# bennyguo/instant-nsr-pl

Hardware: NVIDIA H100
Metric: rays/sec fwd+bwd (NeRF-Synthetic lego shape) (higher is better)
Workload: dtype f16

## Files before the change

include/nsr_b200.h:

```cpp
#ifndef NSR_B200_H
#define NSR_B200_H
#include <stdint.h>

#ifdef __cplusplus
extern "C" {
#endif

#define NSR_MAX_LEVELS 32
#define NSR_VERSION 100

typedef struct {
  int32_t n_levels;
  int32_t n_features;
  float scale[NSR_MAX_LEVELS];
  uint32_t res[NSR_MAX_LEVELS];
  uint32_t size[NSR_MAX_LEVELS];
  uint32_t offset[NSR_MAX_LEVELS];
  uint32_t dense_mask;
} nsr_grid_t;

typedef struct {
  int32_t n_in;
  int32_t n_out;
  int32_t n_hidden;
// ... 131 lines not shown
                             const int64_t* k_dev, const float* xyzdir, void* denc_h, void* stream);
int nsr_nerf_field_bwd_net(const nsr_nerf_t* f, const void* enc_k_h, const void* dparams_h, const void* cparams_h, const float* d_sraw,
                           const float* d_rgb, float* grad_dparams, float* grad_cparams, float loss_scale, const float* amax, int64_t k,
                           const int64_t* k_dev, const float* xyzdir, void* denc_h, void* stream);
int nsr_nerf_table_scatter(const nsr_grid_t* g, const float* xyz, int32_t stride, const void* denc_h, float loss_scale, const float* amax,
                           float* grad_table, int64_t k, const int64_t* k_dev, int32_t level_begin, int32_t level_end, int32_t ctas_per_sm,
                           void* stream);


int nsr_nerf_rays_fwd(const nsr_nerf_t* f, const float* rays, const uint32_t* masks, int32_t words, const float* t_min,
                      const int64_t* offsets_m, const int32_t* order, float step, float early_stop_eps, const void* dparams_h,
                      const void* cparams_h,
                      void* enc_save_h, float* sigmas, float* rgbs, float* weights, float* trans, int32_t* kidx, float* acc_rgb,
                      float* opacity, float* depth, int32_t* kept, uint32_t* ticket, int64_t n_rays, const int32_t* counts,
                      const int32_t* bin_counts, int32_t* kept_blocks, void* stream);
int nsr_nerf_render_rays(const nsr_nerf_t* f, const nsr_march_t* m, const float* rays, const uint32_t* masks, int32_t words,
                         const float* t_start, const int32_t* counts, const int32_t* bin_counts, const int32_t* order_bins,
                         float early_stop_eps, const void* dparams_h, const void* cparams_h, float* acc_rgb, float* opacity,
                         float* depth, int32_t* kept, uint32_t* ticket, int64_t n_rays, void* stream);
int nsr_pack_kept(const int64_t* offsets_m, const int64_t* offsets_k, const float* t_min, float step, const int32_t* kidx,
                  const float* weights, int32_t* ray_indices_k, float* t_starts_k, float* t_ends_k, float* weights_k ,
                  int64_t* loose_pos ,
                  const nsr_nerf_t* f, const float* rays, const void* enc_loose_h ,
                  void* enc_k_h ,
                  float* xyzdir_k ,
                  int32_t enc_tiled ,
                  int64_t n_rays, void* stream);
int nsr_pack_kept_scan(const int64_t* offsets_m, const int32_t* kept, int64_t* offsets_k_out, const float* t_min, float step,
                       const int32_t* kidx, const float* weights, int32_t* ray_indices_k, float* t_starts_k, float* t_ends_k,
                       float* weights_k, int64_t* loose_pos, const nsr_nerf_t* f, const float* rays, const void* enc_loose_h, void* enc_k_h,
                       float* xyzdir_k, int32_t enc_tiled, int64_t n_rays, const int32_t* kept_blocks, void* stream);
int nsr_nerf_ray_bwd_loose(const int64_t* offsets_m, const int32_t* kept, const float* t_min, float step, const int32_t* kidx, const float* trans,
                           const float* weights, const float* sigmas, const float* rgbs, const float* g_rgb, const float* g_opacity,
                           const float* g_depth, const float* g_weights, float* d_sraw, float* d_rgb, float* amax,
                           const int64_t* offsets_k, int64_t n_rays, void* stream);
int nsr_nerf_rays_bwd(const nsr_nerf_t* f, const float* rays, const float* t_min, const int64_t* offsets_m, const int32_t* kept, float step,
                      const void* enc_save_h, const float* sigmas, const float* rgbs, const float* weights, const float* trans,
                      const int32_t* kidx, const void* dparams_h, const void* cparams_h, const float* g_rgb, const float* g_opacity,
                      const float* g_depth, const float* g_weights, float* grad_dparams, float* grad_cparams, float loss_scale, float* amax,
                      float t_bound, uint32_t* ticket, int64_t n_rays, void* stream);
int nsr_neus_field_fwd(const nsr_grid_t* g, const float* points, const void* table_h, const float* W1, const float* b1, const float* W2,
                       const float* b2, float radius, int32_t n_out, float* sdf, float* grad, float* feature, int64_t n, const int64_t* n_dev,
                       void* stream);
int nsr_neus_field_bwd(const nsr_grid_t* g, const float* points, const void* table_h, const float* W1, const float* b1, const float* W2,
                       const float* b2, float radius, int32_t n_out, const float* g_out, const float* g_sdf, const float* g_grad,
                       const float* amax, float* grad_table, float* dW1, float* db1, float* dW2, float* db2, int64_t n, const int64_t* n_dev,
                       void* stream);
int nsr_neus_field_fwd_levels(const nsr_grid_t* g, const float* points, const void* table_h, const float* W1, const float* b1, const float* W2,
                              const float* b2, float radius, int32_t n_out, const float* n_active, float* sdf, float* grad, float* feature, int64_t n,
                              const int64_t* n_dev, void* stream);
// ... 119 lines not shown
```

instant-nsr-pl_b200/csrc/nerf_rays_fwd.cu:

```cuda
#include "march.cuh"
#include "nerf_fused.cuh"

namespace {

constexpr int kWarps = 8;
constexpr int kThreads = kWarps * 32;
constexpr int kMaxWords = 64;
constexpr int kMaxWordsCone = 96;
constexpr int kWarpHalves = 32 * NF_LD32 + 32 * 24 + 64 + 256;
constexpr size_t kSmemBytes = (size_t)(NF_W_TOTAL + kWarps * kWarpHalves) * sizeof(__half);

struct RaysFwdArgs {
  const float* rays;
  const uint32_t* masks;
  const float* t_min;
  const int64_t* offsets_m;
  const int32_t* order;
  const int32_t* bin_counts;
  const int32_t* counts;
  const __half* dparams;
  const __half* cparams;
  __half* enc_save;
  float* sigmas;
  float* rgbs;
  float* weights;
  float* trans;
  int32_t* kidx_out;
  float* acc_rgb;
  float* opacity;
  float* depth;
  int32_t* kept;
  int32_t* kept_blocks;
  uint32_t* ticket;
  float step, early_stop_eps;
  int words;
  int64_t n_rays;
  float cone;
};

__device__ __forceinline__ float warp_incl_prod(float v, int lane) {
#pragma unroll
  for (int o = 1; o < 32; o <<= 1) {
    const float t = __shfl_up_sync(0xffffffffu, v, o);
    if (lane >= o) v *= t;
  }
  return v;
}
// ... 1 lines not shown
#pragma unroll
  for (int o = 16; o > 0; o >>= 1) v += __shfl_xor_sync(0xffffffffu, v, o);
  return v;
}

constexpr int kMinBlocks = 2;
constexpr int kGatherBatch = 4;
template <bool CONE, bool STORE>
__global__ void __launch_bounds__(kThreads, kMinBlocks) nerf_rays_fwd_kernel(const __grid_constant__ nsr_nerf_t P, const RaysFwdArgs a) {
  extern __shared__ __align__(16) __half smem[];
  const int warp = threadIdx.x >> 5, lane = threadIdx.x & 31, g = lane >> 2, c = lane & 3;
  __half* At = smem + NF_W_TOTAL + warp * kWarpHalves;
  __half* St = At + 32 * NF_LD32;
  float* s_sig = reinterpret_cast<float*>(St + 32 * 24);
  float* s_rgb = s_sig + 32;
  const __half2* table = reinterpret_cast<const __half2*>(a.dparams + NF_DENSITY_PARAMS);
  nf_stage_weights(smem, a.dparams, a.cparams, true);
  __shared__ int bins[NSR_ORDER_BINS];
  if (threadIdx.x < NSR_ORDER_BINS) bins[threadIdx.x] = a.bin_counts != nullptr ? __ldg(a.bin_counts + threadIdx.x) : 0;
  __syncthreads();

  for (;;) {
    int64_t ray = 0;
    if (lane == 0) ray = atomicAdd(a.ticket, 1u);
    ray = __shfl_sync(0xffffffffu, ray, 0);
    if (ray >= a.n_rays) break;
    if (a.bin_counts != nullptr) {
      int t = (int)ray, b = 0;
#pragma unroll
      for (int q = 0; q < NSR_ORDER_BINS - 1; ++q) {
// ... 63 lines not shown
          filled += take;
        }
        const bool valid = k >= 0;
        if (!valid) k = 0;
        const float t0 = CONE ? ct0 : __fmaf_rn((float)k, a.step, tmin), t1 = CONE ? ct1 : __fmaf_rn((float)k + 1.f, a.step, tmin);
        const float mid = (t0 + t1) * 0.5f;
        uint32_t f[16];
        if (valid && CONE) {
          float x = fmaf(dx, mid, ox), y = fmaf(dy, mid, oy), z = fmaf(dz, mid, oz);
          nf_contract<NF_UNBOUNDED_SPHERE>(P, x, y, z);
          nf_gather_batched<16, kGatherBatch>(P.grid, table, x, y, z, f);
        } else if (valid) {
          const float x = (fmaf(dx, mid, ox) + P.radius) * inv, y = (fmaf(dy, mid, oy) + P.radius) * inv,
                      z = (fmaf(dz, mid, oz) + P.radius) * inv;
          nf_gather_batched<16, kGatherBatch>(P.grid, table, x, y, z, f);
        } else {
#pragma unroll
          for (int l = 0; l < 16; ++l) f[l] = 0u;
        }
        nf_store_row32(At, lane, f);
        if (STORE && a.enc_save != nullptr && valid) {
          uint4* e = reinterpret_cast<uint4*>(a.enc_save + (base + s_idx) * 32);
          e[0] = make_uint4(f[0], f[1], f[2], f[3]);
          e[1] = make_uint4(f[4], f[5], f[6], f[7]);
          e[2] = make_uint4(f[8], f[9], f[10], f[11]);
          e[3] = make_uint4(f[12], f[13], f[14], f[15]);
        }
        __syncwarp();
        uint32_t a_o[2][1][4];
        {
// ... 67 lines not shown
          d_acc += w * mid;
          r_acc += w * cr;
          g_acc += w * cg;
          b_acc += w * cb;
          if (STORE) {
            const int64_t p = base + s_idx;
            a.sigmas[p] = sigma;
            a.weights[p] = w;
            a.trans[p] = T;
            a.kidx_out[p] = k;
            a.rgbs[p * 3 + 0] = cr;
            a.rgbs[p * 3 + 1] = cg;
            a.rgbs[p * 3 + 2] = cb;
          }
        }
        kept += __popc(__ballot_sync(0xffffffffu, keep));
        carry *= __shfl_sync(0xffffffffu, incl, 31);
        __syncwarp();
        if (carry < a.early_stop_eps) break;
      }
    }
    o_acc = warp_sum(o_acc);
    d_acc = warp_sum(d_acc);
    r_acc = warp_sum(r_acc);
    g_acc = warp_sum(g_acc);
    b_acc = warp_sum(b_acc);
    if (lane == 0) {
      a.opacity[ray] = o_acc;
      a.depth[ray] = d_acc;
      a.acc_rgb[ray * 3 + 0] = r_acc;
      a.acc_rgb[ray * 3 + 1] = g_acc;
// ... 72 lines not shown
    for (int64_t v = lane; v < cnt * 4; v += 32) {
      const int64_t R = dst + (v >> 2);
      const int kc = (int)(v & 3), r = (int)(R & 127);
      enc_k[(R >> 7) * 512 + ((r >> 3) * 4 + kc) * 8 + (r & 7)] = enc_loose[src * 4 + v];
    }
  }
}

__global__ void __launch_bounds__(256) ray_bwd_loose_kernel(const int64_t* __restrict__ off_m, const int32_t* __restrict__ kept,
                                                            const float* __restrict__ t_min, float step, const int32_t* __restrict__ kidx,
                                                            const float* __restrict__ trans, const float* __restrict__ weights,
                                                            const float* __restrict__ sigmas, const float* __restrict__ rgbs,
                                                            const float* __restrict__ g_rgb, const float* __restrict__ g_opacity,
                                                            const float* __restrict__ g_depth, const float* __restrict__ g_weights,
                                                            float* __restrict__ d_sraw, float* __restrict__ d_rgb, float* __restrict__ amax,
                                                            const int64_t* __restrict__ off_k, int64_t n_rays) {
  const int lane = threadIdx.x & 31;
  const int64_t ray = blockIdx.x * 8ll + (threadIdx.x >> 5);
  if (ray >= n_rays) return;
  const int64_t beg = off_m[ray];
  const int64_t out0 = off_k ? off_k[ray] : beg;
  const int n = kept[ray];
  if (n <= 0) return;
  const float tmin = t_min[ray];
  const float gr = g_rgb ? g_rgb[ray * 3 + 0] : 0.f, gg = g_rgb ? g_rgb[ray * 3 + 1] : 0.f, gb = g_rgb ? g_rgb[ray * 3 + 2] : 0.f;
  const float go = g_opacity ? g_opacity[ray] : 0.f, gd = g_depth ? g_depth[ray] : 0.f;
  float carry = 0.f, vmax = 0.f;
  for (int cb = ((n - 1) / 32) * 32; cb >= 0; cb -= 32) {
    const int j = cb + lane;
    const bool ok = j < n;
    const int64_t i = beg + j;
    float w = 0.f, gi = 0.f, delta = 0.f;
    if (ok) {
      w = weights[i];
      const float kf = (float)kidx[i];
      const float t0 = __fmaf_rn(kf, step, tmin), t1 = __fmaf_rn(kf + 1.f, step, tmin);
      delta = t1 - t0;
      gi = gr * rgbs[i * 3 + 0] + gg * rgbs[i * 3 + 1] + gb * rgbs[i * 3 + 2] + go + gd * ((t0 + t1) * 0.5f) + (g_weights ? g_weights[i] : 0.f);
      d_rgb[(out0 + j) * 3 + 0] = w * gr;
      d_rgb[(out0 + j) * 3 + 1] = w * gg;
      d_rgb[(out0 + j) * 3 + 2] = w * gb;
      vmax = fmaxf(vmax, 0.25f * w * fmaxf(fabsf(gr), fmaxf(fabsf(gg), fabsf(gb))));
    }
    const float gw = gi * w;
    float suf = gw;
#pragma unroll
    for (int o = 1; o < 32; o <<= 1) {
      const float t = __shfl_down_sync(0xffffffffu, suf, o);
      if (lane + o < 32) suf += t;
    }
    if (ok) {
      const float ds = delta * (gi * (trans[i] - w) - (carry + suf - gw));
      const float dr = ds * fminf(sigmas[i], 3269017.37f);
      d_sraw[out0 + j] = dr;
      vmax = fmaxf(vmax, fabsf(dr));
    }
    carry += __shfl_sync(0xffffffffu, suf, 0);
  }
  if (amax != nullptr) {
#pragma unroll
    for (int o = 16; o > 0; o >>= 1) vmax = fmaxf(vmax, __shfl_xor_sync(0xffffffffu, vmax, o));
    if (lane == 0 && vmax > 0.f && isfinite(vmax)) atomicMax(reinterpret_cast<int*>(amax), __float_as_int(vmax));
  }
}

template <bool CONE, bool STORE>
int reserve_smem(const char* name) {
  static thread_local bool attr_set = false;
  if (!attr_set) {
    cudaError_t e = cudaFuncSetAttribute(nerf_rays_fwd_kernel<CONE, STORE>, cudaFuncAttributeMaxDynamicSharedMemorySize, (int)kSmemBytes);
    if (e != cudaSuccess) {
      nsr_set_error("%s: cannot reserve %zu B shared memory: %s", name, kSmemBytes, cudaGetErrorString(e));
      return 2;
    }
    attr_set = true;
  }
  return 0;
}

int rays_grid(int64_t n_rays) {
  const int64_t want = (n_rays + kWarps - 1) / kWarps;
  return (int)min((int64_t)nsr_sm_count() * 2, want > 0 ? want : (int64_t)1);
}

}

extern "C" int nsr_nerf_rays_fwd(const nsr_nerf_t* f, const float* rays, const uint32_t* masks, int32_t words, const float* t_min,
                                 const int64_t* offsets_m, const int32_t* order, float step, float early_stop_eps, const void* dparams_h, const void* cparams_h,
                                 void* enc_save_h, float* sigmas, float* rgbs, float* weights, float* trans, int32_t* kidx,
                                 float* acc_rgb, float* opacity, float* depth, int32_t* kept, uint32_t* ticket, int64_t n_rays,
                                 const int32_t* counts, const int32_t* bin_counts, int32_t* kept_blocks, void* stream) {
  NSR_REQUIRE(bin_counts == nullptr || (order != nullptr && counts != nullptr), "nsr_nerf_rays_fwd: the binned queue needs order [8][n] and counts");
  NSR_REQUIRE(f != nullptr && f->grid.n_levels == 16 && f->grid.n_features == 2 && f->feature_dim == 16 && f->density_hidden == 1 &&
                  f->color_hidden == 2 && f->contraction == 0,
              "nsr_nerf_rays_fwd: fused path needs L=16, F=2, feature_dim=16, hidden layers 1/2, AABB contraction");
  NSR_REQUIRE(words >= 1 && words <= kMaxWords, "nsr_nerf_rays_fwd: words must be in [1,%d]", kMaxWords);
  NSR_REQUIRE(ticket != nullptr && kept != nullptr, "nsr_nerf_rays_fwd: ticket / kept are required");
  if (n_rays == 0) return 0;
  if (int e = reserve_smem<false, true>("nsr_nerf_rays_fwd")) return e;
  RaysFwdArgs a;
  a.rays = rays; a.masks = masks; a.t_min = t_min; a.offsets_m = offsets_m; a.order = order; a.bin_counts = bin_counts; a.counts = counts; a.kept_blocks = kept_blocks;
  a.dparams = (const __half*)dparams_h; a.cparams = (const __half*)cparams_h; a.enc_save = (__half*)enc_save_h;
  a.sigmas = sigmas; a.rgbs = rgbs; a.weights = weights; a.trans = trans; a.kidx_out = kidx;
  a.acc_rgb = acc_rgb; a.opacity = opacity; a.depth = depth; a.kept = kept; a.ticket = ticket;
  a.step = step; a.early_stop_eps = early_stop_eps; a.words = words; a.n_rays = n_rays; a.cone = 0.f;
  nerf_rays_fwd_kernel<false, true><<<rays_grid(n_rays), kThreads, kSmemBytes, (cudaStream_t)stream>>>(*f, a);
  NSR_CHECK_LAUNCH("nsr_nerf_rays_fwd");
  return 0;
}

extern "C" int nsr_nerf_render_rays(const nsr_nerf_t* f, const nsr_march_t* m, const float* rays, const uint32_t* masks, int32_t words,
                                    const float* t_start, const int32_t* counts, const int32_t* bin_counts, const int32_t* order_bins,
                                    float early_stop_eps, const void* dparams_h, const void* cparams_h, float* acc_rgb, float* opacity,
                                    float* depth, int32_t* kept, uint32_t* ticket, int64_t n_rays, void* stream) {
  NSR_REQUIRE(f != nullptr && m != nullptr, "nsr_nerf_render_rays: field / march descriptor is NULL");
  NSR_REQUIRE(f->grid.n_levels == 16 && f->grid.n_features == 2 && f->feature_dim == 16 && f->density_hidden == 1 && f->color_hidden == 2,
              "nsr_nerf_render_rays: needs L=16, F=2, feature_dim=16, hidden layers 1/2");
  NSR_REQUIRE(f->contraction == m->contraction, "nsr_nerf_render_rays: field contraction %d != march contraction %d", f->contraction,
              m->contraction);
  NSR_REQUIRE(f->contraction == NF_AABB || f->contraction == NF_UNBOUNDED_SPHERE,
              "nsr_nerf_render_rays: contraction type %d not implemented (AABB=0, UN_BOUNDED_SPHERE=2)", f->contraction);
  const bool cone = f->contraction == NF_UNBOUNDED_SPHERE;
  NSR_REQUIRE(m->step > 0.f && (cone ? m->cone_angle >= 0.f : m->cone_angle == 0.f),
// ... 56 lines not shown
  dummy.radius = 1.f;
  pack_kept_kernel<true><<<nsr_blocks(n_rays, 8), 256, 0, (cudaStream_t)stream>>>(offsets_m, nullptr, kept, offsets_k_out, t_min, step, kidx, weights,
                                                                                  ray_indices_k, t_starts_k, t_ends_k, weights_k, loose_pos,
                                                                                  f ? *f : dummy, rays, (const uint4*)enc_loose_h,
                                                                                  (uint4*)enc_k_h, xyzdir_k, enc_tiled, n_rays, kept_blocks);
  NSR_CHECK_LAUNCH("nsr_pack_kept_scan");
  return 0;
}

extern "C" int nsr_nerf_ray_bwd_loose(const int64_t* offsets_m, const int32_t* kept, const float* t_min, float step, const int32_t* kidx,
                                      const float* trans, const float* weights, const float* sigmas, const float* rgbs, const float* g_rgb,
                                      const float* g_opacity, const float* g_depth, const float* g_weights, float* d_sraw, float* d_rgb,
                                      float* amax, const int64_t* offsets_k, int64_t n_rays, void* stream) {
  if (n_rays == 0) return 0;
  ray_bwd_loose_kernel<<<nsr_blocks(n_rays, 8), 256, 0, (cudaStream_t)stream>>>(offsets_m, kept, t_min, step, kidx, trans, weights, sigmas, rgbs,
                                                                                g_rgb, g_opacity, g_depth, g_weights, d_sraw, d_rgb, amax, offsets_k, n_rays);
  NSR_CHECK_LAUNCH("nsr_nerf_ray_bwd_loose");
  return 0;
}
```

instant-nsr-pl_b200/fused.py:

```python
import ctypes
import math

import torch

from . import ops
from .lib import lib, ptr, stream, check_cuda, contig, NerfT
from .nerfacc import ContractionType, ray_aabb_intersect

SCATTER_LEVEL_GROUPS = ((12, 16), (8, 12), (0, 8))


class _NerfRender(torch.autograd.Function):

    @staticmethod
    def forward(ctx, fused, rays, jitter, static, *params):
        kp = fused.kernel_params(*params)
        st = fused.trace(rays, jitter, static, kp)
        n_rays, cap = rays.shape[0], st['cap']
        dev = rays.device
        acc_rgb = torch.zeros(n_rays, 3, device=dev)
        opacity = torch.zeros(n_rays, 1, device=dev)
        depth = torch.zeros(n_rays, 1, device=dev)
        sig = torch.empty(cap, device=dev)
        rgbs = torch.empty(cap, 3, device=dev)
# ... 37 lines not shown
        n = rays.shape[0]
        cap = n * fused.cap_per_ray
        mref = ctypes.byref(fused.march)
        u = None
        if m.randomized:
            u = torch.rand(n, device=dev) if jitter is None else contig(jitter.to(dev), torch.float32)
        grid = m.occupancy_grid
        bits, coarse = grid.bits(), grid.coarse_bits()
        i32 = lambda k: torch.empty(k, dtype=torch.int32, device=dev)
        f32 = lambda *k: torch.empty(*k, dtype=torch.float32, device=dev)
        i64 = lambda k: torch.empty(k, dtype=torch.int64, device=dev)
        words = (fused.cap_per_ray + 31) // 32
        need_grad = (dparams.requires_grad or cparams.requires_grad) and fused._want_grad
        masks, t_min, counts = i32(n * words), f32(n), i32(n)
        nb = (n + 255) // 256
        zz = torch.zeros(12 + nb, dtype=torch.int32, device=dev)
        tick, amax0, m_total, bin_counts = zz[0:1], zz[1:2].view(torch.float32), zz[2:4].view(torch.int64), zz[4:12]
        kept_blocks = zz[12:] if fused.fuse_kept_scan else None
        if fused.march_alloc:
            offsets_m, order = i64(n), i32(8 * n)
            lib.call('nsr_march_rays_alloc', mref, ptr(rays), ptr(u), ptr(bits), ptr(coarse), ptr(masks), words, ptr(t_min), ptr(counts), ptr(offsets_m),
                     ptr(m_total), ptr(bin_counts), ptr(order), n, stream())
        else:
            offsets_m, order = i64(n + 1), i32(n)
            lib.call('nsr_march_rays_mask', mref, ptr(rays), ptr(u), ptr(bits), ptr(coarse), ptr(masks), words, ptr(t_min), ptr(counts), n, stream())
            lib.call('nsr_scan_counts_order', ptr(counts), ptr(offsets_m), ptr(order), n, stream())
            m_total = offsets_m[n:]
        enc = torch.empty(cap, 32, dtype=torch.float16, device=dev) if need_grad else None
        sig, rgbs, weights, trans, kidx = f32(cap), f32(cap, 3), f32(cap), f32(cap), i32(cap)
        acc_rgb, opacity, depth, kept = f32(n, 3), f32(n, 1), f32(n, 1), i32(n)
        offsets_k = i64(n + 1)
        dh, ch = fused.dparams_half(), fused.cparams_half()
        step = float(m.render_step_size)
        lib.call('nsr_nerf_rays_fwd', fused.ref(), ptr(rays), ptr(masks), words, ptr(t_min), ptr(offsets_m), ptr(order), step,
                 float(fused.early_stop_eps), ptr(dh), ptr(ch), ptr(enc), ptr(sig), ptr(rgbs), ptr(weights), ptr(trans), ptr(kidx),
                 ptr(acc_rgb), ptr(opacity), ptr(depth), ptr(kept), ptr(tick), n, ptr(counts), ptr(bin_counts) if fused.march_alloc else None, ptr(kept_blocks), stream())
        if not fused.fuse_kept_scan:
            lib.call('nsr_scan_counts', ptr(kept), ptr(offsets_k), n, stream())
        ri, ts, te, pos = i32(cap), f32(cap), f32(cap), i64(cap)
        packed_bwd = need_grad and fused.bwd_kernel in ('tiles', 'tiles_split', 'tc') and fused.packed_bwd_inputs
        tiled = 1 if fused.bwd_kernel == 'tc' else 0
        pad = 256 - cap % 128 if tiled else 64
        enc_k = torch.empty(cap + pad, 32, dtype=torch.float16, device=dev) if packed_bwd else None
        xyzdir = f32(cap + pad, 6) if packed_bwd else None
        if fused.fuse_kept_scan:
            lib.call('nsr_pack_kept_scan', ptr(offsets_m), ptr(kept), ptr(offsets_k), ptr(t_min), step, ptr(kidx), ptr(weights), ptr(ri), ptr(ts),
                     ptr(te), None, ptr(pos), fused.ref(), ptr(rays), ptr(enc), ptr(enc_k), ptr(xyzdir), tiled, n, ptr(kept_blocks), stream())
        else:
            lib.call('nsr_pack_kept', ptr(offsets_m), ptr(offsets_k), ptr(t_min), step, ptr(kidx), ptr(weights), ptr(ri), ptr(ts), ptr(te), None,
                     ptr(pos), fused.ref(), ptr(rays), ptr(enc), ptr(enc_k), ptr(xyzdir), tiled, n, stream())
        ctx.fused, ctx.n_rays, ctx.cap = fused, n, cap
        ctx.set_materialize_grads(False)
        if packed_bwd:
            enc = None
        ctx.save_for_backward(rays, t_min, offsets_m, offsets_k, kept, enc, sig, rgbs, weights, trans, kidx, ri, ts, te, pos, dh, ch,
                              enc_k, xyzdir, amax0)
        ctx.mark_non_differentiable(ri, ts, te, pos, offsets_m, offsets_k, m_total, counts)
        return acc_rgb, opacity, depth, weights, ri, ts, te, pos, offsets_m, offsets_k, m_total, counts

    @staticmethod
    def backward(ctx, g_rgb, g_op, g_depth, g_w, *_):
        fused = ctx.fused
        rays, t_min, offsets_m, offsets_k, kept, enc, sig, rgbs, weights, trans, kidx, ri, ts, te, pos, dh, ch, enc_k, xyzdir, amax0 = ctx.saved_tensors
        dev = rays.device
        n, cap = ctx.n_rays, ctx.cap
        step = float(fused.model.render_step_size)
        direct = fused.direct_grads
        if direct is not None:
            gd, gc = direct
        else:
            gd = torch.empty(fused.n_dparams, device=dev)
            gc = torch.empty(fused.n_cparams, device=dev)
        n_head = fused.net.mlp.n_params
        split = fused.bwd_kernel == 'tiles_split' and enc_k is not None and n > 0
        (gd[:n_head] if split else gd).zero_()
        gc.zero_()
        if (enc is not None or enc_k is not None) and n > 0:
            f32 = lambda t: None if t is None else contig(t, torch.float32)
            amax = amax0
            if fused.bwd_kernel == 'rays':
                tick = torch.zeros(1, dtype=torch.int32, device=dev)
                lib.call('nsr_nerf_rays_bwd', fused.ref(), ptr(rays), ptr(t_min), ptr(offsets_m), ptr(kept), step, ptr(enc), ptr(sig), ptr(rgbs),
                         ptr(weights), ptr(trans), ptr(kidx), ptr(dh), ptr(ch), ptr(f32(g_rgb)), ptr(f32(g_op)), ptr(f32(g_depth)),
                         ptr(f32(g_w)), ptr(gd), ptr(gc), float(fused.loss_scale), ptr(amax), float(fused.t_bound), ptr(tick), n, stream())
            else:
                packed = enc_k is not None
                pad = 256 - cap % 128 if fused.bwd_kernel == 'tc' else 64
                d_sraw = torch.empty(cap + pad, device=dev)
                d_rgb = torch.empty(cap + pad, 3, device=dev)
                lib.call('nsr_nerf_ray_bwd_loose', ptr(offsets_m), ptr(kept), ptr(t_min), step, ptr(kidx), ptr(trans), ptr(weights), ptr(sig),
                         ptr(rgbs), ptr(f32(g_rgb)), ptr(f32(g_op)), ptr(f32(g_depth)), ptr(f32(g_w)), ptr(d_sraw), ptr(d_rgb), ptr(amax),
                         ptr(offsets_k) if packed else None, n, stream())
                if packed and fused.bwd_kernel == 'tc':
                    if fused._tc_status is None or fused._tc_status.device != dev:
                        fused._tc_status = torch.zeros(1, dtype=torch.int32, device=dev)
                    lib.call('nsr_nerf_field_bwd_tc', fused.ref(), ptr(enc_k), ptr(dh), ptr(ch), ptr(d_sraw), ptr(d_rgb), ptr(gd), ptr(gc),
                             float(fused.loss_scale), ptr(amax), cap, ptr(offsets_k[n:]), ptr(xyzdir), ptr(fused._tc_status), stream())
                elif packed and fused.bwd_kernel == 'tiles_split':
                    denc = torch.empty(cap, 32, dtype=torch.float16, device=dev)
                    lib.call('nsr_nerf_field_bwd_net', fused.ref(), ptr(enc_k), ptr(dh), ptr(ch), ptr(d_sraw), ptr(d_rgb), ptr(gd), ptr(gc),
                             float(fused.loss_scale), ptr(amax), cap, ptr(offsets_k[n:]), ptr(xyzdir), ptr(denc), stream())
                    groups = fused.level_groups or SCATTER_LEVEL_GROUPS
                    off = fused.grid.offset
                    if sorted(l for g in groups for l in range(*g)) != list(range(len(off) - 1)):
                        raise ValueError(f'level_groups {groups} must partition the {len(off) - 1} levels: the backward zeroes the table per group')
                    for gi, (l0, l1) in enumerate(groups):
                        gd[n_head + 2 * int(off[l0]):n_head + 2 * int(off[l1])].zero_()
                        lib.call('nsr_nerf_table_scatter', ctypes.byref(fused.struct.grid), ptr(xyzdir), 6, ptr(denc), float(fused.loss_scale), ptr(amax),
                                 ptr(gd[n_head:]), cap, ptr(offsets_k[n:]), l0, l1, 4 if (fused.exchange_hook is not None and gi > 0) else 0,
                                 stream())
                        if fused.exchange_hook is not None:
                            fused.exchange_hook(gi)
                else:
                    lib.call('nsr_nerf_field_bwd', fused.ref(), ptr(rays), ptr(ri), ptr(ts), ptr(te), ptr(enc_k if packed else enc), ptr(dh), ptr(ch),
                             ptr(d_sraw), ptr(d_rgb), ptr(gd), ptr(gc), float(fused.loss_scale), ptr(amax), cap, ptr(offsets_k[n:]),
                             None if packed else ptr(pos), ptr(xyzdir), stream())
        if direct is not None:
            return None, None, None, None, None
        return gd, gc, None, None, None


def nerf_field_struct(grid, radius, density_bias, contraction_type):
    s = NerfT()
    s.grid = grid.struct
# ... 349 lines not shown
```

instant-nsr-pl_b200/lib.py:

```python
import ctypes as C
import os

import torch

HERE = os.path.dirname(os.path.abspath(__file__))
NSR_MAX_LEVELS = 32


class NsrError(RuntimeError):
    pass


def library_path():
    return os.path.join(HERE, 'libnsr_b200.so')


class GridT(C.Structure):
    _fields_ = [('n_levels', C.c_int32), ('n_features', C.c_int32),
                ('scale', C.c_float * NSR_MAX_LEVELS), ('res', C.c_uint32 * NSR_MAX_LEVELS),
                ('size', C.c_uint32 * NSR_MAX_LEVELS), ('offset', C.c_uint32 * NSR_MAX_LEVELS),
                ('dense_mask', C.c_uint32)]


class MlpT(C.Structure):
# ... 44 lines not shown
    'nsr_scan_counts': [P, P, I64, P],
    'nsr_march_write': [P, P, P, P, P, P, P, P, P, P, I64, P],
    'nsr_visibility': [P, P, P, P, P, F32, F32, I64, P],
    'nsr_weight_from_density_fwd': [P, P, P, P, P, P, I64, P],
    'nsr_weight_from_density_bwd': [P, P, P, P, P, P, P, I64, P],
    'nsr_weight_from_alpha_fwd': [P, P, P, P, I64, P],
    'nsr_weight_from_alpha_bwd': [P, P, P, P, P, P, I64, P],
    'nsr_accumulate': [P, P, P, P, I32, I64, P],
    'nsr_march_rays_mask': [P, P, P, P, P, P, I32, P, P, I64, P],
    'nsr_scan_counts_order': [P, P, P, I64, P],
    'nsr_march_rays_alloc': [P, P, P, P, P, P, I32, P, P, P, P, P, P, I64, P],
    'nsr_march_rays_expand': [P, P, I32, P, P, P, P, P, I64, P],
    'nsr_march_cone_mask': [P, P, P, P, P, F32, F32, P, P, I32, P, P, I64, P],
    'nsr_march_cone_expand': [P, P, I32, P, P, P, P, P, I64, P, I64, P],
    'nsr_nerf_rays_fwd': [P, P, P, I32, P, P, P, F32, F32, P, P, P, P, P, P, P, P, P, P, P, P, P, I64, P, P, P, P],
    'nsr_nerf_render_rays': [P, P, P, P, I32, P, P, P, P, F32, P, P, P, P, P, P, P, I64, P],
    'nsr_pack_kept': [P, P, P, F32, P, P, P, P, P, P, P, P, P, P, P, P, I32, I64, P],
    'nsr_pack_kept_scan': [P, P, P, P, F32, P, P, P, P, P, P, P, P, P, P, P, P, I32, I64, P, P],
    'nsr_nerf_ray_bwd_loose': [P, P, P, F32, P, P, P, P, P, P, P, P, P, P, P, P, P, I64, P],
    'nsr_nerf_rays_bwd': [P, P, P, P, P, F32, P, P, P, P, P, P, P, P, P, P, P, P, P, P, F32, P, F32, P, I64, P],
    'nsr_neus_field_fwd': [P, P, P, P, P, P, P, F32, I32, P, P, P, I64, P, P],
    'nsr_neus_field_bwd': [P, P, P, P, P, P, P, F32, I32, P, P, P, P, P, P, P, P, P, I64, P, P],
    'nsr_neus_field_fwd_levels': [P, P, P, P, P, P, P, F32, I32, P, P, P, P, I64, P, P],
    'nsr_neus_field_bwd_levels': [P, P, P, P, P, P, P, F32, I32, P, P, P, P, P, P, P, P, P, P, I64, P, P],
    'nsr_neus_field_fd_fwd': [P, P, P, P, P, P, P, F32, I32, P, P, P, P, P, I64, P, P],
    'nsr_neus_field_fd_bwd': [P, P, P, P, P, P, P, F32, I32, P, P, P, P, P, P, P, P, P, P, I64, P, P],
    'nsr_neus_sdf_lattice': [P, P, P, P, I32, I32, I32, I32, I32, P, P, P, P, P, F32, I32, P, P, P],
    'nsr_absmax3': [P, I64, P, I64, P, I64, P, I64, P, P],
    'nsr_sample_points': [P, P, P, P, P, P, P, I64, P, P],
    'nsr_neus_alpha_fwd': [P, P, P, P, P, F32, P, P, P, I64, P, P],
    'nsr_neus_alpha_bwd': [P, P, P, P, P, F32, P, P, P, P, P, P, I64, P, P],
    'nsr_neus_composite_fwd': [P, P, P, P, P, P, P, P, P, P, P, P, I64, P],
    'nsr_neus_composite_bwd': [P, P, P, P, P, P, P, P, P, P, P, P, P, P, P, P, I64, P],
    'nsr_neus_render_rays': [P, P, P, I32, P, P, P, P, F32, P, P, P, P, P, F32, I32, P, P, I32, P, P, P, P, P, P, P, P, P, I64, P],
# ... 134 lines not shown
```

Baseline: 15.21 million.

## Write packed backward inputs directly from forward kernel via atomic row allocation

```diff
diff --git a/include/nsr_b200.h b/include/nsr_b200.h
--- a/include/nsr_b200.h
+++ b/include/nsr_b200.h
@@ -169,6 +169,12 @@
                       void* enc_save_h, float* sigmas, float* rgbs, float* weights, float* trans, int32_t* kidx, float* acc_rgb,
                       float* opacity, float* depth, int32_t* kept, uint32_t* ticket, int64_t n_rays, const int32_t* counts,
                       const int32_t* bin_counts, int32_t* kept_blocks, void* stream);
+int nsr_nerf_rays_fwd_rows(const nsr_nerf_t* f, const float* rays, const uint32_t* masks, int32_t words, const float* t_min,
+                           const int64_t* offsets_m, const int32_t* order, float step, float early_stop_eps, const void* dparams_h,
+                           const void* cparams_h, float* sigmas, float* rgbs, float* weights, float* trans, int32_t* kidx, float* acc_rgb,
+                           float* opacity, float* depth, int32_t* kept, uint32_t* ticket, int64_t n_rays, const int32_t* counts,
+                           const int32_t* bin_counts, int32_t* kept_blocks, void* enc_k_h, float* xyzdir, int32_t* row_of_loose,
+                           int64_t* row_count, void* stream);
 int nsr_nerf_render_rays(const nsr_nerf_t* f, const nsr_march_t* m, const float* rays, const uint32_t* masks, int32_t words,
                          const float* t_start, const int32_t* counts, const int32_t* bin_counts, const int32_t* order_bins,
                          float early_stop_eps, const void* dparams_h, const void* cparams_h, float* acc_rgb, float* opacity,
@@ -189,6 +195,10 @@
                            const float* weights, const float* sigmas, const float* rgbs, const float* g_rgb, const float* g_opacity,
                            const float* g_depth, const float* g_weights, float* d_sraw, float* d_rgb, float* amax,
                            const int64_t* offsets_k, int64_t n_rays, void* stream);
+int nsr_nerf_ray_bwd_rows(const int64_t* offsets_m, const int32_t* kept, const float* t_min, float step, const int32_t* kidx, const float* trans,
+                          const float* weights, const float* sigmas, const float* rgbs, const float* g_rgb, const float* g_opacity,
+                          const float* g_depth, const float* g_weights, float* d_sraw, float* d_rgb, float* amax,
+                          const int32_t* row_of_loose, int64_t n_rays, void* stream);
 int nsr_nerf_rays_bwd(const nsr_nerf_t* f, const float* rays, const float* t_min, const int64_t* offsets_m, const int32_t* kept, float step,
                       const void* enc_save_h, const float* sigmas, const float* rgbs, const float* weights, const float* trans,
                       const int32_t* kidx, const void* dparams_h, const void* cparams_h, const float* g_rgb, const float* g_opacity,
diff --git a/instant-nsr-pl_b200/csrc/nerf_rays_fwd.cu b/instant-nsr-pl_b200/csrc/nerf_rays_fwd.cu
--- a/instant-nsr-pl_b200/csrc/nerf_rays_fwd.cu
+++ b/instant-nsr-pl_b200/csrc/nerf_rays_fwd.cu
@@ -7,7 +7,7 @@
 constexpr int kThreads = kWarps * 32;
 constexpr int kMaxWords = 64;
 constexpr int kMaxWordsCone = 96;
-constexpr int kWarpHalves = 32 * NF_LD32 + 32 * 24 + 64 + 256;
+constexpr int kWarpHalves = 32 * NF_LD32 + 32 * 24 + 64 + 256 + 192;
 constexpr size_t kSmemBytes = (size_t)(NF_W_TOTAL + kWarps * kWarpHalves) * sizeof(__half);
 
 struct RaysFwdArgs {
@@ -31,6 +31,10 @@
   float* depth;
   int32_t* kept;
   int32_t* kept_blocks;
+  uint4* enc_k;
+  float* xyzdir;
+  int32_t* row_of_loose;
+  unsigned long long* row_count;
   uint32_t* ticket;
   float step, early_stop_eps;
   int words;
@@ -62,6 +66,7 @@
   __half* St = At + 32 * NF_LD32;
   float* s_sig = reinterpret_cast<float*>(St + 32 * 24);
   float* s_rgb = s_sig + 32;
+  float* s_xyz = s_rgb + 128;
   const __half2* table = reinterpret_cast<const __half2*>(a.dparams + NF_DENSITY_PARAMS);
   nf_stage_weights(smem, a.dparams, a.cparams, true);
   __shared__ int bins[NSR_ORDER_BINS];
@@ -155,6 +160,11 @@
           const float x = (fmaf(dx, mid, ox) + P.radius) * inv, y = (fmaf(dy, mid, oy) + P.radius) * inv,
                       z = (fmaf(dz, mid, oz) + P.radius) * inv;
           nf_gather_batched<16, kGatherBatch>(P.grid, table, x, y, z, f);
+          if (STORE && a.row_count != nullptr) {
+            s_xyz[lane] = x;
+            s_xyz[32 + lane] = y;
+            s_xyz[64 + lane] = z;
+          }
         } else {
 #pragma unroll
           for (int l = 0; l < 16; ++l) f[l] = 0u;
@@ -252,7 +262,27 @@
             a.rgbs[p * 3 + 2] = cb;
           }
         }
-        kept += __popc(__ballot_sync(0xffffffffu, keep));
+        const uint32_t keep_m = __ballot_sync(0xffffffffu, keep);
+        kept += __popc(keep_m);
+        if (STORE && a.row_count != nullptr && keep_m != 0u) {
+          uint32_t r0 = 0u;
+          if (lane == 0) r0 = (uint32_t)atomicAdd(a.row_count, (unsigned long long)__popc(keep_m));
+          r0 = __shfl_sync(0xffffffffu, r0, 0);
+          if (keep) {
+            const uint32_t row = r0 + __popc(keep_m & ((1u << lane) - 1u));
+            a.row_of_loose[base + s_idx] = (int32_t)row;
+            float* o = a.xyzdir + (size_t)row * 6;
+            o[0] = s_xyz[lane]; o[1] = s_xyz[32 + lane]; o[2] = s_xyz[64 + lane]; o[3] = dx; o[4] = dy; o[5] = dz;
+          }
+#pragma unroll
+          for (int v = lane; v < 128; v += 32) {
+            const int src = v >> 2;
+            if ((keep_m >> src) & 1u) {
+              const uint32_t row = r0 + __popc(keep_m & ((1u << src) - 1u));
+              a.enc_k[(size_t)row * 4 + (v & 3)] = reinterpret_cast<const uint4*>(At + src * NF_LD32)[v & 3];
+            }
+          }
+        }
         carry *= __shfl_sync(0xffffffffu, incl, 31);
         __syncwarp();
         if (carry < a.early_stop_eps) break;
@@ -355,7 +385,8 @@
                                                             const float* __restrict__ g_rgb, const float* __restrict__ g_opacity,
                                                             const float* __restrict__ g_depth, const float* __restrict__ g_weights,
                                                             float* __restrict__ d_sraw, float* __restrict__ d_rgb, float* __restrict__ amax,
-                                                            const int64_t* __restrict__ off_k, int64_t n_rays) {
+                                                            const int64_t* __restrict__ off_k, const int32_t* __restrict__ row_of_loose,
+                                                            int64_t n_rays) {
   const int lane = threadIdx.x & 31;
   const int64_t ray = blockIdx.x * 8ll + (threadIdx.x >> 5);
   if (ray >= n_rays) return;
@@ -372,15 +403,16 @@
     const bool ok = j < n;
     const int64_t i = beg + j;
     float w = 0.f, gi = 0.f, delta = 0.f;
+    const int64_t o = !ok ? 0 : row_of_loose ? (int64_t)row_of_loose[i] : out0 + j;
     if (ok) {
       w = weights[i];
       const float kf = (float)kidx[i];
       const float t0 = __fmaf_rn(kf, step, tmin), t1 = __fmaf_rn(kf + 1.f, step, tmin);
       delta = t1 - t0;
       gi = gr * rgbs[i * 3 + 0] + gg * rgbs[i * 3 + 1] + gb * rgbs[i * 3 + 2] + go + gd * ((t0 + t1) * 0.5f) + (g_weights ? g_weights[i] : 0.f);
-      d_rgb[(out0 + j) * 3 + 0] = w * gr;
-      d_rgb[(out0 + j) * 3 + 1] = w * gg;
-      d_rgb[(out0 + j) * 3 + 2] = w * gb;
+      d_rgb[o * 3 + 0] = w * gr;
+      d_rgb[o * 3 + 1] = w * gg;
+      d_rgb[o * 3 + 2] = w * gb;
       vmax = fmaxf(vmax, 0.25f * w * fmaxf(fabsf(gr), fmaxf(fabsf(gg), fabsf(gb))));
     }
     const float gw = gi * w;
@@ -393,7 +425,7 @@
     if (ok) {
       const float ds = delta * (gi * (trans[i] - w) - (carry + suf - gw));
       const float dr = ds * fminf(sigmas[i], 3269017.37f);
-      d_sraw[out0 + j] = dr;
+      d_sraw[o] = dr;
       vmax = fmaxf(vmax, fabsf(dr));
     }
     carry += __shfl_sync(0xffffffffu, suf, 0);
@@ -424,6 +456,31 @@
   return (int)min((int64_t)nsr_sm_count() * 2, want > 0 ? want : (int64_t)1);
 }
 
+int rays_fwd_launch(const nsr_nerf_t* f, const float* rays, const uint32_t* masks, int32_t words, const float* t_min, const int64_t* offsets_m,
+                    const int32_t* order, float step, float early_stop_eps, const void* dparams_h, const void* cparams_h, void* enc_save_h,
+                    float* sigmas, float* rgbs, float* weights, float* trans, int32_t* kidx, float* acc_rgb, float* opacity, float* depth,
+                    int32_t* kept, uint32_t* ticket, int64_t n_rays, const int32_t* counts, const int32_t* bin_counts, int32_t* kept_blocks,
+                    void* enc_k_h, float* xyzdir, int32_t* row_of_loose, int64_t* row_count, void* stream, const char* who) {
+  NSR_REQUIRE(bin_counts == nullptr || (order != nullptr && counts != nullptr), "%s: the binned queue needs order [8][n] and counts", who);
+  NSR_REQUIRE(f != nullptr && f->grid.n_levels == 16 && f->grid.n_features == 2 && f->feature_dim == 16 && f->density_hidden == 1 &&
+                  f->color_hidden == 2 && f->contraction == 0,
+              "%s: fused path needs L=16, F=2, feature_dim=16, hidden layers 1/2, AABB contraction", who);
+  NSR_REQUIRE(words >= 1 && words <= kMaxWords, "%s: words must be in [1,%d]", who, kMaxWords);
+  NSR_REQUIRE(ticket != nullptr && kept != nullptr, "%s: ticket / kept are required", who);
+  if (n_rays == 0) return 0;
+  if (int e = reserve_smem<false, true>(who)) return e;
+  RaysFwdArgs a;
+  a.rays = rays; a.masks = masks; a.t_min = t_min; a.offsets_m = offsets_m; a.order = order; a.bin_counts = bin_counts; a.counts = counts; a.kept_blocks = kept_blocks;
+  a.dparams = (const __half*)dparams_h; a.cparams = (const __half*)cparams_h; a.enc_save = (__half*)enc_save_h;
+  a.sigmas = sigmas; a.rgbs = rgbs; a.weights = weights; a.trans = trans; a.kidx_out = kidx;
+  a.acc_rgb = acc_rgb; a.opacity = opacity; a.depth = depth; a.kept = kept; a.ticket = ticket;
+  a.enc_k = (uint4*)enc_k_h; a.xyzdir = xyzdir; a.row_of_loose = row_of_loose; a.row_count = (unsigned long long*)row_count;
+  a.step = step; a.early_stop_eps = early_stop_eps; a.words = words; a.n_rays = n_rays; a.cone = 0.f;
+  nerf_rays_fwd_kernel<false, true><<<rays_grid(n_rays), kThreads, kSmemBytes, (cudaStream_t)stream>>>(*f, a);
+  NSR_CHECK_LAUNCH(who);
+  return 0;
+}
+
 }
 
 extern "C" int nsr_nerf_rays_fwd(const nsr_nerf_t* f, const float* rays, const uint32_t* masks, int32_t words, const float* t_min,
@@ -431,23 +488,22 @@
                                  void* enc_save_h, float* sigmas, float* rgbs, float* weights, float* trans, int32_t* kidx,
                                  float* acc_rgb, float* opacity, float* depth, int32_t* kept, uint32_t* ticket, int64_t n_rays,
                                  const int32_t* counts, const int32_t* bin_counts, int32_t* kept_blocks, void* stream) {
-  NSR_REQUIRE(bin_counts == nullptr || (order != nullptr && counts != nullptr), "nsr_nerf_rays_fwd: the binned queue needs order [8][n] and counts");
-  NSR_REQUIRE(f != nullptr && f->grid.n_levels == 16 && f->grid.n_features == 2 && f->feature_dim == 16 && f->density_hidden == 1 &&
-                  f->color_hidden == 2 && f->contraction == 0,
-              "nsr_nerf_rays_fwd: fused path needs L=16, F=2, feature_dim=16, hidden layers 1/2, AABB contraction");
-  NSR_REQUIRE(words >= 1 && words <= kMaxWords, "nsr_nerf_rays_fwd: words must be in [1,%d]", kMaxWords);
-  NSR_REQUIRE(ticket != nullptr && kept != nullptr, "nsr_nerf_rays_fwd: ticket / kept are required");
-  if (n_rays == 0) return 0;
-  if (int e = reserve_smem<false, true>("nsr_nerf_rays_fwd")) return e;
-  RaysFwdArgs a;
-  a.rays = rays; a.masks = masks; a.t_min = t_min; a.offsets_m = offsets_m; a.order = order; a.bin_counts = bin_counts; a.counts = counts; a.kept_blocks = kept_blocks;
-  a.dparams = (const __half*)dparams_h; a.cparams = (const __half*)cparams_h; a.enc_save = (__half*)enc_save_h;
-  a.sigmas = sigmas; a.rgbs = rgbs; a.weights = weights; a.trans = trans; a.kidx_out = kidx;
-  a.acc_rgb = acc_rgb; a.opacity = opacity; a.depth = depth; a.kept = kept; a.ticket = ticket;
-  a.step = step; a.early_stop_eps = early_stop_eps; a.words = words; a.n_rays = n_rays; a.cone = 0.f;
-  nerf_rays_fwd_kernel<false, true><<<rays_grid(n_rays), kThreads, kSmemBytes, (cudaStream_t)stream>>>(*f, a);
-  NSR_CHECK_LAUNCH("nsr_nerf_rays_fwd");
-  return 0;
+  return rays_fwd_launch(f, rays, masks, words, t_min, offsets_m, order, step, early_stop_eps, dparams_h, cparams_h, enc_save_h, sigmas, rgbs,
+                         weights, trans, kidx, acc_rgb, opacity, depth, kept, ticket, n_rays, counts, bin_counts, kept_blocks, nullptr, nullptr,
+                         nullptr, nullptr, stream, "nsr_nerf_rays_fwd");
+}
+
+extern "C" int nsr_nerf_rays_fwd_rows(const nsr_nerf_t* f, const float* rays, const uint32_t* masks, int32_t words, const float* t_min,
+                                      const int64_t* offsets_m, const int32_t* order, float step, float early_stop_eps, const void* dparams_h,
+                                      const void* cparams_h, float* sigmas, float* rgbs, float* weights, float* trans, int32_t* kidx,
+                                      float* acc_rgb, float* opacity, float* depth, int32_t* kept, uint32_t* ticket, int64_t n_rays,
+                                      const int32_t* counts, const int32_t* bin_counts, int32_t* kept_blocks, void* enc_k_h, float* xyzdir,
+                                      int32_t* row_of_loose, int64_t* row_count, void* stream) {
+  NSR_REQUIRE(enc_k_h != nullptr && xyzdir != nullptr && row_of_loose != nullptr && row_count != nullptr,
+              "nsr_nerf_rays_fwd_rows: enc_k / xyzdir / row_of_loose / row_count is NULL");
+  return rays_fwd_launch(f, rays, masks, words, t_min, offsets_m, order, step, early_stop_eps, dparams_h, cparams_h, nullptr, sigmas, rgbs,
+                         weights, trans, kidx, acc_rgb, opacity, depth, kept, ticket, n_rays, counts, bin_counts, kept_blocks, enc_k_h, xyzdir,
+                         row_of_loose, row_count, stream, "nsr_nerf_rays_fwd_rows");
 }
 
 extern "C" int nsr_nerf_render_rays(const nsr_nerf_t* f, const nsr_march_t* m, const float* rays, const uint32_t* masks, int32_t words,
@@ -534,7 +590,21 @@
                                       float* amax, const int64_t* offsets_k, int64_t n_rays, void* stream) {
   if (n_rays == 0) return 0;
   ray_bwd_loose_kernel<<<nsr_blocks(n_rays, 8), 256, 0, (cudaStream_t)stream>>>(offsets_m, kept, t_min, step, kidx, trans, weights, sigmas, rgbs,
-                                                                                g_rgb, g_opacity, g_depth, g_weights, d_sraw, d_rgb, amax, offsets_k, n_rays);
+                                                                                g_rgb, g_opacity, g_depth, g_weights, d_sraw, d_rgb, amax, offsets_k, nullptr,
+                                                                                n_rays);
   NSR_CHECK_LAUNCH("nsr_nerf_ray_bwd_loose");
   return 0;
 }
+
+extern "C" int nsr_nerf_ray_bwd_rows(const int64_t* offsets_m, const int32_t* kept, const float* t_min, float step, const int32_t* kidx,
+                                     const float* trans, const float* weights, const float* sigmas, const float* rgbs, const float* g_rgb,
+                                     const float* g_opacity, const float* g_depth, const float* g_weights, float* d_sraw, float* d_rgb,
+                                     float* amax, const int32_t* row_of_loose, int64_t n_rays, void* stream) {
+  NSR_REQUIRE(row_of_loose != nullptr, "nsr_nerf_ray_bwd_rows: row_of_loose is NULL");
+  if (n_rays == 0) return 0;
+  ray_bwd_loose_kernel<<<nsr_blocks(n_rays, 8), 256, 0, (cudaStream_t)stream>>>(offsets_m, kept, t_min, step, kidx, trans, weights, sigmas, rgbs,
+                                                                                g_rgb, g_opacity, g_depth, g_weights, d_sraw, d_rgb, amax, nullptr,
+                                                                                row_of_loose, n_rays);
+  NSR_CHECK_LAUNCH("nsr_nerf_ray_bwd_rows");
+  return 0;
+}
diff --git a/instant-nsr-pl_b200/fused.py b/instant-nsr-pl_b200/fused.py
--- a/instant-nsr-pl_b200/fused.py
+++ b/instant-nsr-pl_b200/fused.py
@@ -75,9 +75,10 @@
         need_grad = (dparams.requires_grad or cparams.requires_grad) and fused._want_grad
         masks, t_min, counts = i32(n * words), f32(n), i32(n)
         nb = (n + 255) // 256
-        zz = torch.zeros(12 + nb, dtype=torch.int32, device=dev)
+        zz = torch.zeros(14 + nb, dtype=torch.int32, device=dev)
         tick, amax0, m_total, bin_counts = zz[0:1], zz[1:2].view(torch.float32), zz[2:4].view(torch.int64), zz[4:12]
-        kept_blocks = zz[12:] if fused.fuse_kept_scan else None
+        row_count = zz[12:14].view(torch.int64)
+        kept_blocks = zz[14:] if fused.fuse_kept_scan else None
         if fused.march_alloc:
             offsets_m, order = i64(n), i32(8 * n)
             lib.call('nsr_march_rays_alloc', mref, ptr(rays), ptr(u), ptr(bits), ptr(coarse), ptr(masks), words, ptr(t_min), ptr(counts), ptr(offsets_m),
@@ -87,42 +88,51 @@
             lib.call('nsr_march_rays_mask', mref, ptr(rays), ptr(u), ptr(bits), ptr(coarse), ptr(masks), words, ptr(t_min), ptr(counts), n, stream())
             lib.call('nsr_scan_counts_order', ptr(counts), ptr(offsets_m), ptr(order), n, stream())
             m_total = offsets_m[n:]
-        enc = torch.empty(cap, 32, dtype=torch.float16, device=dev) if need_grad else None
+        packed_bwd = need_grad and fused.bwd_kernel in ('tiles', 'tiles_split', 'tc') and fused.packed_bwd_inputs
+        fwd_rows = packed_bwd and fused.bwd_kernel == 'tiles_split'
+        tiled = 1 if fused.bwd_kernel == 'tc' else 0
+        pad = 256 - cap % 128 if tiled else 64
+        enc_k = torch.empty(cap + pad, 32, dtype=torch.float16, device=dev) if packed_bwd else None
+        xyzdir = f32(cap + pad, 6) if packed_bwd else None
+        row_of_loose = i32(cap) if fwd_rows else None
+        enc = torch.empty(cap, 32, dtype=torch.float16, device=dev) if need_grad and not fwd_rows else None
         sig, rgbs, weights, trans, kidx = f32(cap), f32(cap, 3), f32(cap), f32(cap), i32(cap)
         acc_rgb, opacity, depth, kept = f32(n, 3), f32(n, 1), f32(n, 1), i32(n)
         offsets_k = i64(n + 1)
         dh, ch = fused.dparams_half(), fused.cparams_half()
         step = float(m.render_step_size)
-        lib.call('nsr_nerf_rays_fwd', fused.ref(), ptr(rays), ptr(masks), words, ptr(t_min), ptr(offsets_m), ptr(order), step,
-                 float(fused.early_stop_eps), ptr(dh), ptr(ch), ptr(enc), ptr(sig), ptr(rgbs), ptr(weights), ptr(trans), ptr(kidx),
-                 ptr(acc_rgb), ptr(opacity), ptr(depth), ptr(kept), ptr(tick), n, ptr(counts), ptr(bin_counts) if fused.march_alloc else None, ptr(kept_blocks), stream())
+        fwd_args = (fused.ref(), ptr(rays), ptr(masks), words, ptr(t_min), ptr(offsets_m), ptr(order), step, float(fused.early_stop_eps), ptr(dh),
+                    ptr(ch))
+        out_args = (ptr(sig), ptr(rgbs), ptr(weights), ptr(trans), ptr(kidx), ptr(acc_rgb), ptr(opacity), ptr(depth), ptr(kept), ptr(tick), n,
+                    ptr(counts), ptr(bin_counts) if fused.march_alloc else None, ptr(kept_blocks))
+        if fwd_rows:
+            lib.call('nsr_nerf_rays_fwd_rows', *fwd_args, *out_args, ptr(enc_k), ptr(xyzdir), ptr(row_of_loose), ptr(row_count), stream())
+        else:
+            lib.call('nsr_nerf_rays_fwd', *fwd_args, ptr(enc), *out_args, stream())
         if not fused.fuse_kept_scan:
             lib.call('nsr_scan_counts', ptr(kept), ptr(offsets_k), n, stream())
         ri, ts, te, pos = i32(cap), f32(cap), f32(cap), i64(cap)
-        packed_bwd = need_grad and fused.bwd_kernel in ('tiles', 'tiles_split', 'tc') and fused.packed_bwd_inputs
-        tiled = 1 if fused.bwd_kernel == 'tc' else 0
-        pad = 256 - cap % 128 if tiled else 64
-        enc_k = torch.empty(cap + pad, 32, dtype=torch.float16, device=dev) if packed_bwd else None
-        xyzdir = f32(cap + pad, 6) if packed_bwd else None
+        enc_p, enc_kp, xyzdir_p = (None, None, None) if fwd_rows else (enc, enc_k, xyzdir)
         if fused.fuse_kept_scan:
             lib.call('nsr_pack_kept_scan', ptr(offsets_m), ptr(kept), ptr(offsets_k), ptr(t_min), step, ptr(kidx), ptr(weights), ptr(ri), ptr(ts),
-                     ptr(te), None, ptr(pos), fused.ref(), ptr(rays), ptr(enc), ptr(enc_k), ptr(xyzdir), tiled, n, ptr(kept_blocks), stream())
+                     ptr(te), None, ptr(pos), fused.ref(), ptr(rays), ptr(enc_p), ptr(enc_kp), ptr(xyzdir_p), tiled, n, ptr(kept_blocks), stream())
         else:
             lib.call('nsr_pack_kept', ptr(offsets_m), ptr(offsets_k), ptr(t_min), step, ptr(kidx), ptr(weights), ptr(ri), ptr(ts), ptr(te), None,
-                     ptr(pos), fused.ref(), ptr(rays), ptr(enc), ptr(enc_k), ptr(xyzdir), tiled, n, stream())
+                     ptr(pos), fused.ref(), ptr(rays), ptr(enc_p), ptr(enc_kp), ptr(xyzdir_p), tiled, n, stream())
         ctx.fused, ctx.n_rays, ctx.cap = fused, n, cap
         ctx.set_materialize_grads(False)
         if packed_bwd:
             enc = None
         ctx.save_for_backward(rays, t_min, offsets_m, offsets_k, kept, enc, sig, rgbs, weights, trans, kidx, ri, ts, te, pos, dh, ch,
-                              enc_k, xyzdir, amax0)
+                              enc_k, xyzdir, amax0, row_of_loose, row_count)
         ctx.mark_non_differentiable(ri, ts, te, pos, offsets_m, offsets_k, m_total, counts)
         return acc_rgb, opacity, depth, weights, ri, ts, te, pos, offsets_m, offsets_k, m_total, counts
 
     @staticmethod
     def backward(ctx, g_rgb, g_op, g_depth, g_w, *_):
         fused = ctx.fused
-        rays, t_min, offsets_m, offsets_k, kept, enc, sig, rgbs, weights, trans, kidx, ri, ts, te, pos, dh, ch, enc_k, xyzdir, amax0 = ctx.saved_tensors
+        (rays, t_min, offsets_m, offsets_k, kept, enc, sig, rgbs, weights, trans, kidx, ri, ts, te, pos, dh, ch, enc_k, xyzdir, amax0, row_of_loose,
+         row_count) = ctx.saved_tensors
         dev = rays.device
         n, cap = ctx.n_rays, ctx.cap
         step = float(fused.model.render_step_size)
@@ -149,9 +159,12 @@
                 pad = 256 - cap % 128 if fused.bwd_kernel == 'tc' else 64
                 d_sraw = torch.empty(cap + pad, device=dev)
                 d_rgb = torch.empty(cap + pad, 3, device=dev)
-                lib.call('nsr_nerf_ray_bwd_loose', ptr(offsets_m), ptr(kept), ptr(t_min), step, ptr(kidx), ptr(trans), ptr(weights), ptr(sig),
-                         ptr(rgbs), ptr(f32(g_rgb)), ptr(f32(g_op)), ptr(f32(g_depth)), ptr(f32(g_w)), ptr(d_sraw), ptr(d_rgb), ptr(amax),
-                         ptr(offsets_k) if packed else None, n, stream())
+                ray_args = (ptr(offsets_m), ptr(kept), ptr(t_min), step, ptr(kidx), ptr(trans), ptr(weights), ptr(sig), ptr(rgbs), ptr(f32(g_rgb)),
+                            ptr(f32(g_op)), ptr(f32(g_depth)), ptr(f32(g_w)), ptr(d_sraw), ptr(d_rgb), ptr(amax))
+                if row_of_loose is not None:
+                    lib.call('nsr_nerf_ray_bwd_rows', *ray_args, ptr(row_of_loose), n, stream())
+                else:
+                    lib.call('nsr_nerf_ray_bwd_loose', *ray_args, ptr(offsets_k) if packed else None, n, stream())
                 if packed and fused.bwd_kernel == 'tc':
                     if fused._tc_status is None or fused._tc_status.device != dev:
                         fused._tc_status = torch.zeros(1, dtype=torch.int32, device=dev)
@@ -160,7 +173,7 @@
                 elif packed and fused.bwd_kernel == 'tiles_split':
                     denc = torch.empty(cap, 32, dtype=torch.float16, device=dev)
                     lib.call('nsr_nerf_field_bwd_net', fused.ref(), ptr(enc_k), ptr(dh), ptr(ch), ptr(d_sraw), ptr(d_rgb), ptr(gd), ptr(gc),
-                             float(fused.loss_scale), ptr(amax), cap, ptr(offsets_k[n:]), ptr(xyzdir), ptr(denc), stream())
+                             float(fused.loss_scale), ptr(amax), cap, ptr(row_count), ptr(xyzdir), ptr(denc), stream())
                     groups = fused.level_groups or SCATTER_LEVEL_GROUPS
                     off = fused.grid.offset
                     if sorted(l for g in groups for l in range(*g)) != list(range(len(off) - 1)):
@@ -168,7 +181,7 @@
                     for gi, (l0, l1) in enumerate(groups):
                         gd[n_head + 2 * int(off[l0]):n_head + 2 * int(off[l1])].zero_()
                         lib.call('nsr_nerf_table_scatter', ctypes.byref(fused.struct.grid), ptr(xyzdir), 6, ptr(denc), float(fused.loss_scale), ptr(amax),
-                                 ptr(gd[n_head:]), cap, ptr(offsets_k[n:]), l0, l1, 4 if (fused.exchange_hook is not None and gi > 0) else 0,
+                                 ptr(gd[n_head:]), cap, ptr(row_count), l0, l1, 4 if (fused.exchange_hook is not None and gi > 0) else 0,
                                  stream())
                         if fused.exchange_hook is not None:
                             fused.exchange_hook(gi)
diff --git a/instant-nsr-pl_b200/lib.py b/instant-nsr-pl_b200/lib.py
--- a/instant-nsr-pl_b200/lib.py
+++ b/instant-nsr-pl_b200/lib.py
@@ -82,10 +82,12 @@
     'nsr_march_cone_mask': [P, P, P, P, P, F32, F32, P, P, I32, P, P, I64, P],
     'nsr_march_cone_expand': [P, P, I32, P, P, P, P, P, I64, P, I64, P],
     'nsr_nerf_rays_fwd': [P, P, P, I32, P, P, P, F32, F32, P, P, P, P, P, P, P, P, P, P, P, P, P, I64, P, P, P, P],
+    'nsr_nerf_rays_fwd_rows': [P, P, P, I32, P, P, P, F32, F32, P, P, P, P, P, P, P, P, P, P, P, P, I64, P, P, P, P, P, P, P, P],
     'nsr_nerf_render_rays': [P, P, P, P, I32, P, P, P, P, F32, P, P, P, P, P, P, P, I64, P],
     'nsr_pack_kept': [P, P, P, F32, P, P, P, P, P, P, P, P, P, P, P, P, I32, I64, P],
     'nsr_pack_kept_scan': [P, P, P, P, F32, P, P, P, P, P, P, P, P, P, P, P, P, I32, I64, P, P],
     'nsr_nerf_ray_bwd_loose': [P, P, P, F32, P, P, P, P, P, P, P, P, P, P, P, P, P, I64, P],
+    'nsr_nerf_ray_bwd_rows': [P, P, P, F32, P, P, P, P, P, P, P, P, P, P, P, P, P, I64, P],
     'nsr_nerf_rays_bwd': [P, P, P, P, P, F32, P, P, P, P, P, P, P, P, P, P, P, P, P, P, F32, P, F32, P, I64, P],
     'nsr_neus_field_fwd': [P, P, P, P, P, P, P, F32, I32, P, P, P, I64, P, P],
     'nsr_neus_field_bwd': [P, P, P, P, P, P, P, F32, I32, P, P, P, P, P, P, P, P, P, I64, P, P],
```

After: 15.58 million, median of 6. +2.4%, better.
